# thelondonsmiths/Solex_ser_recon_EN

Hardware: AMD Instinct MI355X
Metric: SER frames/sec end-to-end (decode→clahe) + %HBM roofline, 1/2/4/8 MI355X (higher is better)
Workload: dtype u16

## Files before the change

include/shg_hip.h:

```cpp
#ifndef SHG_HIP_H
#define SHG_HIP_H

#include <stddef.h>
#include <stdint.h>

#ifdef __cplusplus
extern "C" {
#endif

#define SHG_ABI_VERSION 16

#define SHG_E_ARG        (-1)
#define SHG_E_WORKSPACE  (-2)
#define SHG_E_UNSUPPORTED (-3)
#define SHG_E_VALUE      (-4)
#define SHG_E_TYPE       (-5)
#define SHG_E_LINALG     (-6)
#define SHG_E_RUNTIME    (-7)
#define SHG_E_QHULL      (-8)
#define SHG_E_ASSERT     (-9)
#define SHG_E_INDEX      (-10)

typedef void* shg_stream_t;

// ... 239 lines not shown
int shg_flood_stats_f64(const double* image, const double* blurred, int64_t n, double very_bright,
                        double* stats, uint32_t* counts, void* workspace, shg_stream_t stream);
int shg_flood_stats_lerp_f64(const double* image, const double* blurred, int64_t n,
                             const double* order_stats, double gamma, double* stats, uint32_t* counts,
                             void* workspace, shg_stream_t stream);

size_t shg_canny_workspace_bytes(int64_t h, int64_t w);
int shg_canny_masks_f64(const double* blurred, int64_t h, int64_t w, double flood_thresh,
                        const double* host_gauss_weights, int radius, double low, double high,
                        uint8_t* low_mask, uint8_t* high_mask, void* workspace, size_t workspace_bytes,
                        shg_stream_t stream);

size_t shg_edge_components_workspace_bytes(int64_t h, int64_t w);
int shg_edge_components(const uint8_t* low_mask, const uint8_t* high_mask, int64_t h, int64_t w,
                        int32_t* out_idx, int32_t* out_root, int32_t* out_count,
                        void* workspace, size_t workspace_bytes, shg_stream_t stream);

size_t shg_contrast_stats_workspace_bytes(int tiles);
size_t shg_contrast_stats_workspace_bytes_for(int64_t h, int64_t w, int tiles);
int shg_contrast_stats_u16(const uint16_t* frame, int64_t h, int64_t w, int64_t pitch, double clip_limit,
                           int tiles, uint16_t* cl1, int64_t cl1_pitch, const int64_t* ranks_frame2,
                           const int64_t* ranks_cl13, double* out5, void* workspace, size_t workspace_bytes,
                           shg_stream_t stream);
int shg_contrast_products_u16(const uint16_t* frame, int64_t frame_pitch, const uint16_t* cl1, int64_t cl1_pitch,
                              int64_t h, int64_t w, const double* lo_hi6, uint16_t* high_contrast,
                              uint16_t* protus, uint16_t* cc, int64_t dst_pitch, int64_t disc_x0,
                              int64_t disc_y0, int64_t disc_r, shg_stream_t stream);
int shg_contrast_products_vec_fits(const uint16_t* frame, int64_t frame_pitch, const uint16_t* cl1, int64_t cl1_pitch,
                                   int64_t h, int64_t w, const uint16_t* high_contrast, const uint16_t* protus,
                                   const uint16_t* cc, int64_t dst_pitch);

int shg_limb_fused_fits(int64_t sh, int64_t sw, int k);
size_t shg_limb_prepare_workspace_bytes(int64_t sh, int64_t sw, int k);
int shg_limb_prepare(const uint16_t* img, int64_t h, int64_t w, int64_t pitch, int k, const int64_t* host_ranks4, double gamma99,
                     double* packed, const uint32_t** keys_out, void* workspace, size_t workspace_bytes, shg_stream_t stream);
size_t shg_limb_edges_workspace_bytes(int64_t sh, int64_t sw);
int shg_limb_edges(const uint32_t* keys, int64_t sh, int64_t sw, int k, double flood_thresh, const double* host_gauss_weights,
                   int radius, double low, double high, int32_t* comp, void* workspace, size_t workspace_bytes, shg_stream_t stream);


size_t shg_stage_mean_fit_workspace_bytes(int64_t n_frames, int64_t height, int64_t width, int bytes_per_px);
size_t shg_stage_mean_fit_host_bytes(int64_t height, int64_t width);
int shg_stage_mean_fit(const void* stack, int64_t n_frames, int64_t height, int64_t width, int bytes_per_px,
                       int64_t frame_stride_px, const uint64_t* sum_in, const uint16_t* max_in, int64_t n_total,
                       uint16_t* mean_out, uint16_t* max_out, int64_t* host_y12, double* host_p4, double* host_fit,
                       int32_t* host_trace_sharp, uint8_t* host_mask_good, void* workspace, size_t workspace_bytes,
// ... 167 lines not shown
```

solex_ser_recon_en_amd/_lib.py:

```python
import ctypes
import os
from ctypes import c_double, c_int, c_int32, c_int64, c_size_t, c_uint16, c_uint32, c_void_p

import torch

_HERE = os.path.dirname(os.path.abspath(__file__))
LIB_PATH = os.path.join(_HERE, 'csrc', 'libshg_hip.so')

if not os.path.exists(LIB_PATH):
    raise ImportError(
        'libshg_hip.so is missing (%s). Build it with `python -c "import __graft_entry__ as g; g.build()"` or '
        '`make -C solex_ser_recon_en_amd/csrc`. There is no CPU fallback for the SHG hot path.' % LIB_PATH)

lib = ctypes.CDLL(LIB_PATH)

P = c_void_p
PD = ctypes.POINTER(c_double)
PI64 = ctypes.POINTER(c_int64)


class ScanRequest(ctypes.Structure):
    _fields_ = [('struct_bytes', c_uint32), ('start_phase', c_int32),
                ('stack', P), ('n_frames', c_int64), ('height', c_int64), ('width', c_int64), ('frame_stride_px', c_int64),
                ('bytes_per_px', c_int32), ('flip_x', c_int32),
# ... 94 lines not shown
                                  c_int64, P, P]),
    'shg_warp_rows_wide_fits': (c_int, [P, c_int64, c_int64, c_int64, c_double, c_double, c_double, P, c_int64, c_int64, c_int64]),
    'shg_rowpair_logratio_stats': (c_int, [P, c_int64, c_int64, c_int64, c_int64, c_int64, P, P, P, P, P]),
    'shg_rowpair_logratio_stats_mirrored': (c_int, [P, c_int64, c_int64, c_int64, c_int64, c_int64, P, P, P, P, P, P]),
    'shg_line_order_stats_u16': (c_int, [P, c_int64, c_int64, c_int64, c_int, c_int64, c_int64, P, P, P]),
    'shg_scale_rows_u16': (c_int, [P, c_int64, c_int64, c_int64, P, P, P, c_int64, P]),
    'shg_scale_rows_vec_fits': (c_int, [P, c_int64, c_int64, c_int64, P, c_int64]),
    'shg_correlate1d_rows_f64': (c_int, [P, c_int64, c_int64, P, c_int, c_int, P, P]),
    'shg_lin_filter_row_sums': (c_int, [P, c_int64, c_int64, c_int64, P, P, P, P, P, c_int, P, P, P]),
    'shg_lin_filter_apply': (c_int, [P, c_int64, c_int64, c_int64, P, P, P, c_int, c_int, P, P, P, P, c_int, P, c_int64, P]),
    'shg_crop_pad_u16': (c_int, [P, c_int64, c_int64, c_int64, P, c_int64, c_int64, c_int64, c_int64, c_int64,
                                 c_int, P]),
    'shg_clahe_workspace_bytes': (c_size_t, [c_int, c_int]),
    'shg_clahe_workspace_bytes_for': (c_size_t, [c_int64, c_int64, c_int, c_int]),
    'shg_clahe': (c_int, [P, c_int64, c_int64, c_int64, c_int, c_double, c_int, P, c_int64, P, c_size_t, P]),
    'shg_hist': (c_int, [P, c_int64, c_int64, c_int64, c_int, P, P]),
    'shg_select_u16_workspace_bytes': (c_size_t, [c_int]),
    'shg_select_u16': (c_int, [P, c_int64, c_int64, c_int64, ctypes.POINTER(c_int64), c_int, P, P, c_size_t, P]),
    'shg_rescale_u16': (c_int, [P, c_int64, c_int64, c_int64, c_double, c_double, c_double, P, c_int64, P]),
    'shg_rescale_u8': (c_int, [P, c_int64, c_int64, c_int64, c_double, c_double, c_double, P, c_int64, P]),
    'shg_contrast_stats_workspace_bytes': (c_size_t, [c_int]),
    'shg_contrast_stats_workspace_bytes_for': (c_size_t, [c_int64, c_int64, c_int]),
    'shg_contrast_stats_u16': (c_int, [P, c_int64, c_int64, c_int64, c_double, c_int, P, c_int64, P, P, P, P, c_size_t, P]),
    'shg_contrast_products_u16': (c_int, [P, c_int64, P, c_int64, c_int64, c_int64, P, P, P, P, c_int64, c_int64, c_int64, c_int64, P]),
    'shg_contrast_products_vec_fits': (c_int, [P, c_int64, P, c_int64, c_int64, c_int64, P, P, P, c_int64]),
    'shg_fill_disc_u16': (c_int, [P, c_int64, c_int64, c_int64, c_int64, c_int64, c_int64, c_uint16, P, P]),
    'shg_downscale_mean_u16': (c_int, [P, c_int64, c_int64, c_int64, c_int, P, P]),
    'shg_box_blur_f64': (c_int, [P, c_int64, c_int64, c_int, P, P, P]),
    'shg_box_blur_key_f64': (c_int, [P, c_int64, c_int64, c_int, P, P, P, P]),
    'shg_select_keys_workspace_bytes': (c_size_t, [c_int]),
    'shg_select_keys_u32': (c_int, [ctypes.POINTER(c_void_p), c_int64, ctypes.POINTER(c_int64), ctypes.POINTER(c_int), c_int, P, P, c_size_t, P]),
    'shg_select_workspace_bytes': (c_size_t, [c_int]),
    'shg_select_f64': (c_int, [P, c_int64, ctypes.POINTER(c_int64), c_int, P, P, c_size_t, P]),
    'shg_select_multi_f64': (c_int, [ctypes.POINTER(c_void_p), c_int64, ctypes.POINTER(c_int64), c_int, P, P, c_size_t, P]),
    'shg_flood_stats_f64': (c_int, [P, P, c_int64, c_double, P, P, P, P]),
    'shg_flood_stats_lerp_f64': (c_int, [P, P, c_int64, P, c_double, P, P, P, P]),
    'shg_edge_components_workspace_bytes': (c_size_t, [c_int64, c_int64]),
    'shg_edge_components': (c_int, [P, P, c_int64, c_int64, P, P, P, P, c_size_t, P]),
    'shg_canny_workspace_bytes': (c_size_t, [c_int64, c_int64]),
    'shg_canny_masks_f64': (c_int, [P, c_int64, c_int64, c_double, ctypes.POINTER(c_double), c_int, c_double, c_double, P, P, P,
                                    c_size_t, P]),
    'shg_limb_fused_fits': (c_int, [c_int64, c_int64, c_int]),
    'shg_limb_prepare_workspace_bytes': (c_size_t, [c_int64, c_int64, c_int]),
    'shg_limb_prepare': (c_int, [P, c_int64, c_int64, c_int64, c_int, PI64, c_double, P, ctypes.POINTER(c_void_p), P, c_size_t, P]),
    'shg_limb_edges_workspace_bytes': (c_size_t, [c_int64, c_int64]),
    'shg_limb_edges': (c_int, [P, c_int64, c_int64, c_int, c_double, PD, c_int, c_double, c_double, P, P, c_size_t, P]),
# ... 200 lines not shown
```

solex_ser_recon_en_amd/csrc/clahe.hip:

```cpp
#include <stdlib.h>
#include <type_traits>
#include <algorithm>
#include "shg_common.h"

namespace {
template <typename T>
__device__ __forceinline__ T* zdisk(T* p, size_t zs, uint32_t z) {
    return reinterpret_cast<T*>(reinterpret_cast<char*>(const_cast<typename std::remove_const<T>::type*>(p)) + (size_t)z * zs);
}

constexpr int HIST16 = 65536;
constexpr int SEL_SLOTS = 8;
constexpr int SEL_NW = 8;
struct SelWin { uint32_t w0_cur, w0_next, max, pad; };
constexpr int SEL_WIN_SLOTS = 8;
constexpr int SEL_WIN_WORDS = SEL_WIN_SLOTS * SEL_NW * 256;
__device__ __forceinline__ uint32_t sel_window_origin(const SelWin* st) {
    const uint32_t w0 = __hip_atomic_load(&st->w0_cur, __ATOMIC_RELAXED, __HIP_MEMORY_SCOPE_AGENT);
    return w0 > 256u - SEL_NW ? 256u - SEL_NW : w0;
}
constexpr int SLICE_PX = 32768;
constexpr int kFusedMaxSliceRows = 2048;

template <typename T>
// ... 66 lines not shown
    return (uint32_t)min(q, 65535);
}
__device__ __forceinline__ double row_factor_for_fma(double c) {
    if (c != c) return 0.0;
    if (c > 0x1p+960) return 65536.0;
    if (c < -0x1p+960) return -4294967296.0;
    return c;
}

struct HistSlicesArgs {
    shg::PtrBatch imgs;
    int64_t h, w, pitch;
    int tiles;
    int64_t th, tw;
    uint32_t* part;
    size_t zs;
    int slice_rows, vec;
    FusedSrc fs;
    int clip, chunk_rows;
};

__device__ __forceinline__ int64_t mirror101(int64_t i, int64_t n) { return 2 * (n - 1) - i; }

template <bool FUSED, int BITS> __global__ __launch_bounds__(1024) void k_tile_hist16_slices(const HistSlicesArgs kargs) {
    const shg::PtrBatch& imgs = kargs.imgs;
    const int64_t h = kargs.h, w = kargs.w, pitch = kargs.pitch, th = kargs.th, tw = kargs.tw;
    const int tiles = kargs.tiles, slice_rows = kargs.slice_rows, vec = kargs.vec;
    uint32_t* __restrict__ part = kargs.part;
    const size_t zs = kargs.zs;
    const FusedSrc& fs = kargs.fs;
    extern __shared__ uint32_t lh[];
    const uint16_t* __restrict__ img = imgs.at<const uint16_t>(blockIdx.z);
    part = zdisk(part, zs, blockIdx.z);
    const int tile = blockIdx.y;
    const int64_t ty = tile / tiles, tx = tile % tiles;
    const int ya = (int)blockIdx.x * slice_rows;
    const int yb = min((int)th, ya + slice_rows) - 1;
    for (int i = threadIdx.x; i < HIST16 / 8; i += 1024) reinterpret_cast<uint4*>(lh)[i] = make_uint4(0, 0, 0, 0);
    double* cf = reinterpret_cast<double*>(lh + HIST16 / 2);
    const uint16_t* __restrict__ raw = nullptr;
    uint16_t* __restrict__ fin = nullptr;
    __shared__ uint32_t fill_s;
    const bool scaled = FUSED && fs.c != nullptr;
    if (FUSED) {
        raw = fs.raw.at<const uint16_t>(blockIdx.z);
        fin = imgs.at<uint16_t>(blockIdx.z);
        const double* c = scaled ? fs.c + (int64_t)blockIdx.z * h : nullptr;
        for (int i = threadIdx.x; i <= yb - ya; i += 1024) {
            int64_t r = ty * th + ya + i;
            if (r >= h) r = mirror101(r, h);
            cf[i] = scaled ? row_factor_for_fma(c[r]) : 1.0;
        }
        if (threadIdx.x == 0) fill_s = scaled ? scale_px(raw[0], c[0]) : (uint32_t)raw[0];
    }
    __syncthreads();
    const int chunk_rows = BITS == 16 ? slice_rows : kargs.chunk_rows;
    const uint32_t clip2 = (uint32_t)kargs.clip;
    for (int ca = ya; ca <= yb; ca += chunk_rows) {
        const int cb = min(yb, ca + chunk_rows - 1);
        if (BITS != 16 && ca != ya) {
            __syncthreads();
            for (int i = threadIdx.x; i < HIST16 / 8; i += 1024) {
                uint4 q = reinterpret_cast<uint4*>(lh)[i];
                uint32_t* d = reinterpret_cast<uint32_t*>(&q);
#pragma unroll
                for (int j = 0; j < 4; ++j) d[j] = min(d[j] & 0xffffu, clip2) | (min(d[j] >> 16, clip2) << 16);
                reinterpret_cast<uint4*>(lh)[i] = q;
            }
            __syncthreads();
        }
        const int lane = threadIdx.x & 63, wave = threadIdx.x >> 6;
        const int twi = (int)tw;
        const int64_t xbase = tx * tw;
        auto count = [&](uint32_t v) { atomicAdd(&lh[v >> 1], 1u << ((v & 1u) << 4)); };
        if (vec) {
            const int64_t xa = xbase, xb = min(xbase + tw, w);
            const int64_t xa8 = (xa + 7) & ~(int64_t)7, xb8 = max(xb & ~(int64_t)7, xa8);
            const int nvr = (int)((xb8 - xa8) / 8);
            const int n_head = (int)(min(xa8, xb) - xa), n_tail = (int)(xb - max(xb8, xa + n_head)), n_edge = n_head + n_tail + (int)(xbase + tw - xb);
            {
                const uint32_t nvr_u = (uint32_t)nvr, total_v = (uint32_t)(cb - ca + 1) * nvr_u;
                const float inv_nvr = nvr > 0 ? 1.0f / (float)nvr : 0.0f;
                constexpr int U = 4;
                for (uint32_t i0 = threadIdx.x; i0 < total_v; i0 += 1024u * U) {
                    uint4 q[U];
                    int64_t yv[U];
                    uint32_t vv[U], rowv[U];
                    bool borderv[U];
#pragma unroll
                    for (int u = 0; u < U; ++u) {
                        const uint32_t i = i0 + 1024u * u < total_v ? i0 + 1024u * u : i0;
                        uint32_t r = (uint32_t)((float)i * inv_nvr);
                        r -= (r * nvr_u > i) ? 1u : 0u;
                        r += ((r + 1u) * nvr_u <= i) ? 1u : 0u;
                        rowv[u] = r;
                        vv[u] = i - r * nvr_u;
                        int64_t y = ty * th + ca + (int64_t)r;
                        borderv[u] = y >= h;
                        if (borderv[u]) y = mirror101(y, h);
                        yv[u] = y;
                        const uint16_t* srow = FUSED ? raw + y * fs.raw_pitch : img + y * pitch;
                        q[u] = reinterpret_cast<const uint4*>(srow + xa8)[vv[u]];
                    }
#pragma unroll
                    for (int u = 0; u < U; ++u) {
                        if (i0 + 1024u * u >= total_v) break;
                        uint32_t d[4] = {q[u].x, q[u].y, q[u].z, q[u].w};
                        if (FUSED) {
                            if (scaled) {
                                const double cy = cf[ca - ya + (int)rowv[u]], kc = cy * 0x1p+52;
#pragma unroll
                                for (int j = 0; j < 4; ++j) d[j] = (scale_px_fma(d[j] & 0xffffu, cy, kc) & 0xffffu) | (scale_px_fma(d[j] >> 16, cy, kc) << 16);
                            }
                            if (!borderv[u]) reinterpret_cast<uint4*>(fin + yv[u] * pitch + xa8)[vv[u]] = make_uint4(d[0], d[1], d[2], d[3]);
                        }
#pragma unroll
                        for (int j = 0; j < 4; ++j) { count(d[j] & 0xffffu); count(d[j] >> 16); }
                    }
                }
            }
            for (int e = threadIdx.x; e < (cb - ca + 1) * n_edge; e += 1024) {
                const int rr = e / n_edge, l = e - rr * n_edge, yy = ca + rr;
                int64_t y = ty * th + yy;
                const bool border_row = y >= h;
                if (border_row) y = mirror101(y, h);
                const int64_t x = l < n_head ? xa + l : (l < n_head + n_tail ? xb - n_tail + (l - n_head) : xb + (l - n_head - n_tail));
                const bool border_col = x >= w;
                const int64_t xr = border_col ? mirror101(x, w) : x;
                uint32_t v = (FUSED ? raw + y * fs.raw_pitch : img + y * pitch)[xr];
                if (FUSED) {
                    const double cy = cf[yy - ya];
                    if (scaled) v = scale_px_fma(v, cy, cy * 0x1p+52) & 0xffffu;
                    if (!border_col && !border_row) fin[y * pitch + x] = (uint16_t)v;
                }
                count(v);
            }
        } else {
            for (int yy = ca + wave; yy <= cb; yy += 16) {
                int64_t y = ty * th + yy;
                const bool border_row = y >= h;
                if (border_row) y = mirror101(y, h);
                const uint16_t* row = FUSED ? raw + y * fs.raw_pitch : img + y * pitch;
                const double cy = FUSED ? cf[yy - ya] : 1.0, kc = cy * 0x1p+52;
// ... 1324 lines not shown
    bool ranks_done = false;
};

struct SelectRequest {
    Disks disks;
    int64_t h, w, pitch;
    const int64_t* ranks; int n_ranks;
    double* out; int out_zstride;
    void* workspace; size_t workspace_bytes; shg_stream_t stream;
    ClaheResult after = {};
};

enum class Route { Atomics8, Atomics16, Slices16, Slices8, Slices4 };
inline bool is_slices(Route r) { return r >= Route::Slices16; }

struct Plan {
    int err; char msg[120];
    Route route;
    ClaheLayout lay;
    int ntiles, clip;
    int64_t th, tw, area;
    float lut_scale;
    int bits, hist_vec;
    int64_t slice_rows, slices, chunk_rows;
    bool window;
    bool lut_all_tiles;
    int64_t lut_rank[2];
    int blend_px, blend_rounds, blend_tiled;
    bool blend_counts;
    uint32_t blend_tiles_x, blend_blocks;
};

#define PLAN_REQUIRE(cond, code, ...) \
    do { if (!(cond)) { p.err = (code); snprintf(p.msg, sizeof(p.msg), __VA_ARGS__); return p; } } while (0)

inline Plan plan_clahe(const ClaheRequest& r, const Tuning& tune) {
    Plan p = {};
    const Disks& d = r.disks;
    const int64_t h = r.im.h, w = r.im.w, pitch = r.im.pitch, dst_pitch = r.im.dst_pitch;
    const int tiles = r.im.tiles, bytes_per_px = r.im.bytes_per_px;
    PLAN_REQUIRE(h > 0 && w > 0 && pitch >= w && dst_pitch >= w, SHG_E_ARG, "shg_clahe: bad image size");
    PLAN_REQUIRE(bytes_per_px == 1 || bytes_per_px == 2, SHG_E_ARG, "shg_clahe: bytes_per_px must be 1 or 2");
    PLAN_REQUIRE(tiles >= 1 && tiles <= 16, SHG_E_UNSUPPORTED, "shg_clahe: tiles must be in 1..16");
    PLAN_REQUIRE(h < 65536, SHG_E_UNSUPPORTED, "shg_clahe: more than 65535 rows");
    p.lay = clahe_layout(h, w, tiles, bytes_per_px);
    PLAN_REQUIRE(r.workspace_bytes >= p.lay.small, SHG_E_WORKSPACE, "shg_clahe: workspace too small");
// ... 26 lines not shown
    int64_t slice_px = (d.n >= tune.big_from && tune.slice_px > SLICE_PX && tune.slice_px <= 65535) ? tune.slice_px : SLICE_PX;
    if (sat && tune.sat_px) slice_px = tune.sat_px;
    p.chunk_rows = slice_rows_of(tw, 65280);
    p.slice_rows = slice_rows_of(tw, slice_px);
    if (sat) {
        const int64_t max_slices = std::min<int64_t>(256, p.lay.n_slices * (16 / p.bits));
        if (!tune.sat_px) {
            int64_t best = 1, best_cost = INT64_MAX;
            for (int64_t sl = 1; sl <= std::min<int64_t>(max_slices, th); ++sl) {
                const int64_t rows = ceil_div(th, sl);
                if (d.fused && rows > kFusedMaxSliceRows) continue;
                const int64_t cost = ceil_div(ceil_div(th, rows) * p.ntiles * (int64_t)d.n, shg::kCUs) * (rows * tw + 8192);
                if (cost < best_cost) { best_cost = cost; best = rows; }
            }
            p.slice_rows = best;
        }
        if (ceil_div(th, p.slice_rows) > max_slices) p.slice_rows = ceil_div(th, max_slices);
        if (d.fused) p.slice_rows = std::min<int64_t>(p.slice_rows, kFusedMaxSliceRows);
    }
    p.slices = ceil_div(th, p.slice_rows);
    PLAN_REQUIRE(!d.fused || p.slice_rows <= kFusedMaxSliceRows, SHG_E_ARG, "shg_clahe: the fused histogram's slices hold at most %d rows", kFusedMaxSliceRows);
    const uintptr_t ptr_bits = d.bits_of(d.src) | d.bits_of(d.dst);
    p.hist_vec = tw >= 64 && pitch % 8 == 0 && (ptr_bits & 15) == 0 && (!d.fused || d.from_in_vectors(w));
    p.window = r.sel_hist && r.want_window;
    p.lut_all_tiles = p.ntiles <= 16 && d.n >= 8;

    const bool vec = (ptr_bits & 7) == 0 && pitch % 4 == 0 && dst_pitch % 4 == 0;
    p.blend_px = vec ? 4 : 1;
    p.blend_counts = vec && r.sel_hist;
    p.blend_rounds = p.blend_counts ? 4 : 1;
    p.blend_tiles_x = 1u;
    if (p.blend_counts && tune.interp_tiled) {
        const int shape = tune.interp_shape;
        const int lw = shape ? (shape & 15) : 2, wx = shape ? ((shape >> 4) & 15) : 2;
        const bool px8 = (shape ? ((shape >> 8) & 1) != 0 : d.n >= 4) && (ptr_bits & 15) == 0 && pitch % 8 == 0 && dst_pitch % 8 == 0;
        p.blend_px = px8 ? 8 : 4;
        const int64_t wg_px = (int64_t)p.blend_px << (lw + wx), wg_rows = (int64_t)(64 >> lw) * (4 >> wx);
        p.blend_tiles_x = (uint32_t)ceil_div(w, wg_px);
        p.blend_tiled = 0x10000 | lw | (wx << 8);
        p.blend_blocks = p.blend_tiles_x * (uint32_t)ceil_div(h, wg_rows * p.blend_rounds);
    } else {
        p.blend_blocks = (unsigned)ceil_div(ceil_div(w, p.blend_px) * h, 256 * (int64_t)p.blend_rounds);
    }
    return p;
}
#undef PLAN_REQUIRE

template <typename Args> using Kernel = void (*)(Args);
inline Kernel<HistSlicesArgs> pick_hist_slices(bool fused, int bits) {
    if (fused) return bits == 16 ? k_tile_hist16_slices<true, 16> : bits == 8 ? k_tile_hist16_slices<true, 8> : k_tile_hist16_slices<true, 4>;
    return bits == 16 ? k_tile_hist16_slices<false, 16> : bits == 8 ? k_tile_hist16_slices<false, 8> : k_tile_hist16_slices<false, 4>;
}
inline Kernel<HistReduceArgs> pick_hist_reduce(int bits) { return bits == 16 ? k_hist_reduce : bits == 8 ? k_hist_reduce_sat<8> : k_hist_reduce_sat<4>; }
inline Kernel<LutBlocksArgs> pick_lut_blocks(bool sat, bool all_tiles) {
    if (all_tiles) return sat ? k_tile_lut16_blocks<true, true> : k_tile_lut16_blocks<false, true>;
    return sat ? k_tile_lut16_blocks<true, false> : k_tile_lut16_blocks<false, false>;
}
inline Kernel<InterpVmArgs> pick_interp_vm(int px, bool counts, bool t2) {
    if (counts && px == 8) return t2 ? k_clahe_interp_vm<8, true, true> : k_clahe_interp_vm<8, true, false>;
    if (counts) return t2 ? k_clahe_interp_vm<4, true, true> : k_clahe_interp_vm<4, true, false>;
    if (px == 4) return t2 ? k_clahe_interp_vm<4, false, true> : k_clahe_interp_vm<4, false, false>;
    return t2 ? k_clahe_interp_vm<1, false, true> : k_clahe_interp_vm<1, false, false>;
}

void ensure_lds_attr() {
    static const bool done = [] {
        auto allow = [](auto kernel, size_t lds) {
            (void)hipFuncSetAttribute(reinterpret_cast<const void*>(kernel), hipFuncAttributeMaxDynamicSharedMemorySize, (int)lds);
        };
        for (int bits : {16, 8, 4}) {
            allow(pick_hist_slices(false, bits), HIST16 * 2);
            allow(pick_hist_slices(true, bits), HIST16 * 2 + kFusedMaxSliceRows * 8);
        }
        allow(pick_lut_blocks(true, true), 2048 * 16 * 2);
        allow(pick_lut_blocks(false, true), 2048 * 16 * 2);
        allow(k_tile_hist16, HIST16 * 2);
        allow(k_image_hist16, HIST16 * 2);
        allow(k_tile_lut16_lds, (HIST16 + HIST16 / 64) * 2);
        return true;
    }();
    (void)done;
}

ClaheResult clahe_slices(const ClaheRequest& r, const Plan& p) {
    ClaheResult out;
    ensure_lds_attr();
    hipStream_t st = shg::as_stream(r.stream);
    const Disks& d = r.disks;
    const Shape& im = r.im;
    char* ws = static_cast<char*>(r.workspace);
    uint32_t* hist = reinterpret_cast<uint32_t*>(ws);
    uint16_t* lut = reinterpret_cast<uint16_t*>(ws + p.lay.lut);
    uint32_t* part = reinterpret_cast<uint32_t*>(ws + p.lay.slices);
    uint32_t* chunk_tile = reinterpret_cast<uint32_t*>(ws + p.lay.chunk);
    int32_t* se = reinterpret_cast<int32_t*>(ws + p.lay.se);
    const unsigned nz = (unsigned)d.n, ntiles = (unsigned)p.ntiles;
    const bool sat = p.bits != 16;
    { SHG_PROF("clahe_hist", st);
      const HistSlicesArgs ha{d.src, im.h, im.w, im.pitch, im.tiles, p.th, p.tw, part, d.zs, (int)p.slice_rows, p.hist_vec, d.fused ? d.from : FusedSrc{}, p.clip, (int)p.chunk_rows};
      const size_t lds = HIST16 * 2 + (d.fused ? (size_t)p.slice_rows * 8 : 0);
      if ((out.err = shg::launch(pick_hist_slices(d.fused, p.bits), dim3((unsigned)p.slices, ntiles, nz), dim3(1024), lds, st, ha, "k_tile_hist16_slices")))
          return out;
      const HistReduceArgs ra{part, (int)p.slices, p.clip, hist, chunk_tile, se, d.zs, r.sel_hist, r.sel_hist ? SEL_SLOTS * r.sel_stride : 0, p.window ? 1 : 0};
      if ((out.err = shg::launch(pick_hist_reduce(p.bits), dim3(p.bits == 8 ? 64u : 32u, ntiles, nz), dim3(sat ? 256u : 1024u), 0, st, ra, sat ? "k_hist_reduce_sat" : "k_hist_reduce")))
          return out;
      out.sel_zeroed = r.sel_hist != nullptr; }
    { SHG_PROF("clahe_lut", st);
      LutBlocksArgs la{hist, se, p.clip, p.lut_scale, lut, d.zs, 0, {0, 0}, nullptr, 0, nullptr, 0, (int)p.area, p.ntiles, BorderPx{{}, im.h, im.w, im.pitch, im.h, im.w}};
      if (r.ranks) {
          la.border = BorderPx{d.src, im.h, im.w, im.pitch, p.th * im.tiles, p.tw * im.tiles};
          la.n_ranks = 2, la.rank[0] = p.lut_rank[0], la.rank[1] = p.lut_rank[1];
          la.chunk_sums = chunk_tile, la.chunk_sets = p.ntiles;
          la.ranks_out = r.ranks->out, la.ranks_zstride = r.ranks->out_zstride;
          out.ranks_done = true;
      }
      const dim3 grid(32u + (unsigned)la.n_ranks, p.lut_all_tiles ? 1u : ntiles, nz);
      const size_t lds = p.lut_all_tiles ? (size_t)2048 * p.ntiles * sizeof(uint16_t) : 0;
      if ((out.err = shg::launch(pick_lut_blocks(sat, p.lut_all_tiles), grid, dim3(1024), lds, st, la, "k_tile_lut16_blocks"))) return out; }
    { SHG_PROF("clahe_interp", st);
      const InterpVmArgs ia{d.src, im.h, im.w, im.pitch, im.tiles, 1.0f / (float)p.tw, 1.0f / (float)p.th, lut, d.dst, im.dst_pitch, p.blend_rounds,
                            p.blend_counts ? r.sel_hist : nullptr, p.blend_counts ? r.sel_stride : 0, d.zs, p.blend_tiled, p.blend_tiles_x, p.blend_counts && p.window ? 1 : 0};
      if ((out.err = shg::launch(pick_interp_vm(p.blend_px, p.blend_counts, im.tiles == 2), dim3(p.blend_blocks, 1u, nz), dim3(256), 0, st, ia, "k_clahe_interp_vm")))
          return out;
      out.pass0_done = p.blend_counts;
// ... 224 lines not shown
        const RanksJob job{{ranks.v[0], ranks.v[1]}, out5 + 5 * i0, 5};
        ClaheRequest cr{d, Shape{h, w, pitch, cl1_pitch, 2, clip_limit, tiles}, ws, lay.select2, stream};
        cr.want_chunks = true;
        cr.sel_hist = reinterpret_cast<uint32_t*>(ws + lay.select3);
        cr.sel_stride = (1 + 3) * 256;
        cr.want_window = tune.window_for(m);
        cr.ranks = &job;
        const ClaheResult c = clahe_impl(cr, tune);
        if (c.err) return c.err;
        SHG_REQUIRE(c.chunk_tile && c.sel_zeroed, SHG_E_RUNTIME, "shg_contrast_stats_u16: the batched path did not take the slice histograms");
        if (!c.ranks_done) {
            SHG_PROF("hist_ranks", st);
            if (int e = shg::launch(k_hist_ranks, dim3(2u, 1u, (unsigned)m), dim3(1024), 0, st,
                                   HistRanksArgs{reinterpret_cast<const uint32_t*>(ws), c.chunk_tile, tiles * tiles, tiles * tiles, ranks, out5 + 5 * i0, per, 5}, "k_hist_ranks"))
                return e;
        }
        d.src = d.dst;
        SelectRequest sr{d, h, w, cl1_pitch, ranks_cl13, 3, out5 + 5 * i0 + 2, 5, cr.sel_hist, select_bytes(3), stream};
        sr.after = c;
        if (int e = select_u16_impl(sr, tune)) return e;
    }
    return 0;
}
```

solex_ser_recon_en_amd/csrc/transversalium.hip:

```cpp
#include <math.h>
#include <algorithm>
#include "shg_common.h"
#include "fast_log.h"

namespace {

constexpr int MAXN = SHG_TRANSV_MAX_COLS;
constexpr int NT = 256;

using shg::f64_key;
using shg::key_f64;

constexpr int NB = 512;
constexpr int CAP = 128;

struct alignas(16) Scratch {
    uint32_t hist[2][256];
    int64_t wave_tot[2][4];
    int64_t pick[2][3];
    unsigned long long found[2];
    unsigned long long cand[CAP];
    unsigned long long kmin, kmax;
    uint32_t n_cand;
    double red[8];
// ... 159 lines not shown
#pragma unroll
            for (int r = 0; r < 2; ++r) {
                const uint32_t rk = (uint32_t)(r ? rank_hi : rank_lo);
                if (run <= rk && rk < p[7]) {
                    uint32_t b = 0, before = run, in = c[0];
#pragma unroll
                    for (int k = 0; k < 7; ++k) {
                        const bool past = rk >= p[k];
                        b += past ? 1u : 0u;
                        before = past ? p[k] : before;
                        in = past ? c[k + 1] : in;
                    }
                    sc.pick32[4 * r] = 8u * (uint32_t)lane + b;
                    sc.pick32[4 * r + 1] = before;
                    sc.pick32[4 * r + 2] = in;
                }
            }
        }
        __syncthreads();
        const int b0 = (int)sc.pick32[0], b1 = (int)sc.pick32[4];
        const uint32_t base = sc.pick32[1];
        const uint32_t cnt = sc.pick32[2] + (b1 != b0 ? sc.pick32[6] : 0u);
        if (cnt <= (uint32_t)CAP) {
            const double from = b0 == 0 ? -__builtin_huge_val() : (double)b0, to = b1 == NB - 1 ? __builtin_huge_val() : (double)(b1 + 1);
            sweep(n, [&](int i) {
                const double v = val(i);
                const double t = place(v);
                if (in_play(v) && t >= from && t < to) cand[atomicAdd(&sc.n_cand, 1u)] = v;
            });
            __syncthreads();
            const int m = (int)sc.n_cand;
            if (tid < m) {
                const double mine = cand[tid];
                uint32_t r = base;
                for (int j = 0; j < m; ++j) {
                    const double o = cand[j];
                    r += (o < mine || (o == mine && j < tid)) ? 1u : 0u;
                }
                if (r == (uint32_t)rank_lo) sc.vfound[0] = mine;
                if (r == (uint32_t)rank_hi) sc.vfound[1] = mine;
            }
            __syncthreads();
            out_lo = sc.vfound[0];
            out_hi = sc.vfound[1];
            __syncthreads();
            return true;
        }
        if (b0 != b1) return false;
        if (tid == 0) { sc.kmin = ~0ull; sc.kmax = 0ull; }
        __syncthreads();
        uint64_t mn = ~0ull, mx = 0ull;
// ... 154 lines not shown
        }
        if (odd) sc.nonfinite = 1;
    } else {
        bool odd = false;
        for (int i = threadIdx.x; i < n; i += NT) {
            const double q = ((double)r1[i] * f1) / ((double)r0[i] * f0);
            const double x = (q >= 2.2250738585072014e-308 && q <= 1.7976931348623157e308) ? shg::log_normal(q) : log(q);
            if (x != x) sc.bad = 1;
            odd = odd || !(fabs(x) <= 1.7976931348623157e308);
            vals[i] = x;
            sum1 += x;
            sum2 = fma(x, x, sum2);
        }
        if (odd) sc.nonfinite = 1;
    }
    float rough1 = (float)sum1, rough2 = (float)sum2;
    block_sum2_rough(rough1, rough2, sc.redf);
    __syncthreads();
    if (sc.bad) {
        emit(__builtin_nan(""));
        return;
    }
    const bool finite = !sc.nonfinite;
    const float per_n = __builtin_amdgcn_rcpf((float)n);
    const float meanf = rough1 * per_n, varf = rough2 * per_n - meanf * meanf;
    const double mean = (double)meanf;
    const double sigma = varf > 0.0f ? (double)__builtin_amdgcn_sqrtf(varf) : 0.0;
    const int lo = (n & 1) ? (n >> 1) : (n >> 1) - 1, hi = n >> 1;
    double va, vb;
    auto general = [&](auto key) {
        uint64_t ka, kb;
        select2(key, n, lo, hi, sc, ka, kb);
        va = key_f64(ka);
        vb = key_f64(kb);
    };
    const double kMedSpan = 1.0, kMadSpan = 1.0;
    auto row_val = [&](int i) { return vals[i]; };
    if (!(finite && select2_buckets(row_val, n, lo, hi, mean - kMedSpan * sigma, mean + kMedSpan * sigma, sc, va, vb)))
        general([&](int i) { return f64_key(vals[i]); });
    const double med = (n & 1) ? va : (va + vb) / 2.0;
    if (!finite) {
        for (int i = threadIdx.x; i < n; i += NT) {
            const double dv = fabs(vals[i] - med);
            if (dv != dv) sc.bad = 1;
        }
        __syncthreads();
        if (sc.bad) {
            emit(__builtin_nan(""));
            return;
        }
    }
    auto dev_val = [&](int i) { return fabs(vals[i] - med); };
    if (!(finite && select2_buckets(dev_val, n, lo, hi, 0.0, kMadSpan * sigma, sc, va, vb)))
        general([&](int i) { return f64_key(fabs(vals[i] - med)); });
    const double mdev = (n & 1) ? va : (va + vb) / 2.0;
    const double twice = 2.0 * mdev;
    const bool all = !(mdev != 0.0);
    double s = 0.0;
    uint32_t kept = 0;
    sweep<false>(n, [&](int i) {
        const double x = vals[i];
        const bool keep = all || fabs(x - med) < twice;
        kept += (uint32_t)__popcll(__ballot(keep));
        if (keep) s += x;
    });
    s = wave_sum(s);
    __syncthreads();
    if ((threadIdx.x & 63) == 0) { sc.red[threadIdx.x >> 6] = s; sc.kept[threadIdx.x >> 6] = kept; }
    __syncthreads();
    s = (sc.red[0] + sc.red[1]) + (sc.red[2] + sc.red[3]);
    const double cnt = (double)((sc.kept[0] + sc.kept[1]) + (sc.kept[2] + sc.kept[3]));
    emit(s / cnt);
}

__global__ __launch_bounds__(256) void k_scale_rows(shg::PtrBatch imgs, int64_t w, int64_t pitch,
                                                    const double* __restrict__ c, const double* __restrict__ row_factor,
// ... 25 lines not shown
    uint16_t* __restrict__ dst = dsts.at<uint16_t>(blockIdx.z);
    c += (int64_t)blockIdx.z * h;
    const bool factored = row_factor != nullptr;
    const bool full = x + 8 <= w;
    uint4 q[SCALE_ROWS];
    double cy[SCALE_ROWS], fy[SCALE_ROWS];
#pragma unroll
    for (int rr = 0; rr < SCALE_ROWS; ++rr) {
        const int64_t y = ya + rr < h ? ya + rr : h - 1;
        if (full) q[rr] = *reinterpret_cast<const uint4*>(img + y * pitch + x);
        cy[rr] = c[y];
        fy[rr] = factored ? row_factor[y] : 1.0;
    }
#pragma unroll
    for (int rr = 0; rr < SCALE_ROWS; ++rr) {
        const int64_t y = ya + rr;
        if (y >= h) break;
        const double cyr = cy[rr], fyr = fy[rr];
        auto one = [&](uint32_t px) {
            double v = (double)px;
            if (factored) v = v * fyr;
            v = v * cyr;
            v = v > 65535.0 ? 65535.0 : v;
            return (uint32_t)(int)v;
        };
        if (full) {
            uint4 o;
            o.x = one(q[rr].x & 0xffffu) | (one(q[rr].x >> 16) << 16);
            o.y = one(q[rr].y & 0xffffu) | (one(q[rr].y >> 16) << 16);
            o.z = one(q[rr].z & 0xffffu) | (one(q[rr].z >> 16) << 16);
            o.w = one(q[rr].w & 0xffffu) | (one(q[rr].w >> 16) << 16);
            *reinterpret_cast<uint4*>(dst + y * dst_pitch + x) = o;
        } else {
            for (int64_t i = x; i < w; ++i) dst[y * dst_pitch + i] = (uint16_t)one(img[y * pitch + i]);
        }
    }
}

constexpr int CORR_MAXR = 1024;

struct CorrelateArgs {
    const double* src;
    int64_t n;
    const double* weights;
    int radius, symmetric;
    double* dst;
};
// ... 201 lines not shown
```

solex_ser_recon_en_amd/ops.py:

```python
import ctypes

import numpy as np
import torch

from . import _lib
from ._lib import lib


def _stream():
    return torch._C._cuda_getCurrentRawStream(torch.cuda.current_device())


def _dev(t, what):
    if not isinstance(t, torch.Tensor) or not t.is_cuda:
        raise RuntimeError('%s must be a GPU tensor: the SHG hot path has no CPU fallback' % what)
    return t


def _img(t, what, dtype=None):
    _dev(t, what)
    if t.dim() != 2 or (t.shape[1] > 1 and t.stride(1) != 1):
        raise ValueError('%s must be a 2-D image with contiguous rows' % what)
    if dtype is not None and t.dtype != dtype:
        raise TypeError('%s must be %s, got %s' % (what, dtype, t.dtype))
# ... 358 lines not shown
    if need == 0:
        raise ValueError('clahe: unsupported tile count %r' % (tiles,))
    ws = torch.empty(need, dtype=torch.uint8, device=img.device)
    out = pitched_u16(h, w, img.device) if bpp == 2 else torch.empty((h, w), dtype=torch.uint8, device=img.device)
    _lib.check(lib.shg_clahe(ptr, h, w, pitch, bpp, float(clip_limit), int(tiles), out.data_ptr(), out.stride(0),
                             ws.data_ptr(), need, _stream()), 'shg_clahe')
    return out


def contrast_stats_u16(frame, ranks_frame, ranks_cl1, out5, clip_limit=0.8, tiles=2, small_workspace=False):
    import ctypes
    ptr, h, w, pitch = _img(frame, 'frame', torch.uint16)
    need = (lib.shg_contrast_stats_workspace_bytes(int(tiles)) if small_workspace
            else lib.shg_contrast_stats_workspace_bytes_for(h, w, int(tiles)))
    if need == 0:
        raise ValueError('contrast_stats: unsupported tile count %r' % (tiles,))
    ws = torch.empty(need, dtype=torch.uint8, device=frame.device)
    cl1 = pitched_u16(h, w, frame.device)
    rf = (ctypes.c_int64 * 2)(*[int(r) for r in ranks_frame])
    rc = (ctypes.c_int64 * 3)(*[int(r) for r in ranks_cl1])
    _lib.check(lib.shg_contrast_stats_u16(ptr, h, w, pitch, float(clip_limit), int(tiles), cl1.data_ptr(), cl1.stride(0), rf, rc,
                                          out5.data_ptr(), ws.data_ptr(), need, _stream()), 'shg_contrast_stats_u16')
    return cl1


def contrast_products_u16(frame, cl1, lo_hi6, disc=None):
    import ctypes
    ptr, h, w, pitch = _img(frame, 'frame', torch.uint16)
    cptr, ch, cw, cpitch = _img(cl1, 'cl1', torch.uint16)
    if (ch, cw) != (h, w):
        raise ValueError('frame and cl1 must share one shape')
    store = torch.empty((3, h, (w + 63) // 64 * 64), dtype=torch.uint16, device=frame.device)
    hc, protus, cc = store[0, :, :w], store[1, :, :w], store[2, :, :w]
    bounds = (ctypes.c_double * 6)(*[float(v) for v in lo_hi6])
    x0, y0, r = (int(v) for v in disc) if disc is not None else (0, 0, 0)
    _lib.check(lib.shg_contrast_products_u16(ptr, pitch, cptr, cpitch, h, w, bounds, hc.data_ptr(), protus.data_ptr(), cc.data_ptr(),
                                             store.stride(1), x0, y0, r, _stream()), 'shg_contrast_products_u16')
    return hc, protus, cc


def histogram(img):
    _dev(img, 'img')
    bpp = 2 if img.dtype == torch.uint16 else 1
    if img.dtype not in (torch.uint16, torch.uint8):
        raise TypeError('histogram needs uint8 or uint16')
    ptr, h, w, pitch = _img(img, 'img')
# ... 635 lines not shown
```

Baseline: 6.076 million.

## Add early-load fused histogram variant, batched contrast stats API, and NaN-robust median steering

Adds an EARLY variant of the fused CLAHE tile-histogram kernel for small batches (n<=3). It issues the first vector pixel loads before writing row factors to shared memory and hitting the barrier, so that global-load latency overlaps the factor setup. The change also exposes a batched multi-frame contrast-stats entry point with crop and scaling, which lets callers process several frames in one call. Separately, it makes the robust median/MAD selection use bucket steering with finite-only statistics when non-finite values are present, and adjusts bucket boundary and pixel masking semantics. Together these add kernel variants and more surface area to keep correct.

```diff
diff --git a/include/shg_hip.h b/include/shg_hip.h
--- a/include/shg_hip.h
+++ b/include/shg_hip.h
@@ -285,6 +285,11 @@
                            int tiles, uint16_t* cl1, int64_t cl1_pitch, const int64_t* ranks_frame2,
                            const int64_t* ranks_cl13, double* out5, void* workspace, size_t workspace_bytes,
                            shg_stream_t stream);
+int shg_contrast_stats_frames_u16(const uint16_t* const* host_raw, int64_t k, int64_t h, int64_t w, int64_t raw_pitch,
+                                  const double* factors, int64_t out_w, int64_t sx0, int64_t dx0, int64_t ncopy,
+                                  double clip_limit, int tiles, uint16_t* const* host_final, uint16_t* const* host_cl1,
+                                  int64_t out_pitch, const int64_t* ranks_frame2, const int64_t* ranks_cl13, double* out5,
+                                  void* workspace, size_t workspace_bytes, shg_stream_t stream);
 int shg_contrast_products_u16(const uint16_t* frame, int64_t frame_pitch, const uint16_t* cl1, int64_t cl1_pitch,
                               int64_t h, int64_t w, const double* lo_hi6, uint16_t* high_contrast,
                               uint16_t* protus, uint16_t* cc, int64_t dst_pitch, int64_t disc_x0,
diff --git a/solex_ser_recon_en_amd/_lib.py b/solex_ser_recon_en_amd/_lib.py
--- a/solex_ser_recon_en_amd/_lib.py
+++ b/solex_ser_recon_en_amd/_lib.py
@@ -140,6 +140,8 @@
     'shg_contrast_stats_workspace_bytes': (c_size_t, [c_int]),
     'shg_contrast_stats_workspace_bytes_for': (c_size_t, [c_int64, c_int64, c_int]),
     'shg_contrast_stats_u16': (c_int, [P, c_int64, c_int64, c_int64, c_double, c_int, P, c_int64, P, P, P, P, c_size_t, P]),
+    'shg_contrast_stats_frames_u16': (c_int, [P, c_int64, c_int64, c_int64, c_int64, P, c_int64, c_int64, c_int64, c_int64, c_double, c_int,
+                                              P, P, c_int64, P, P, P, P, c_size_t, P]),
     'shg_contrast_products_u16': (c_int, [P, c_int64, P, c_int64, c_int64, c_int64, P, P, P, P, c_int64, c_int64, c_int64, c_int64, P]),
     'shg_contrast_products_vec_fits': (c_int, [P, c_int64, P, c_int64, c_int64, c_int64, P, P, P, c_int64]),
     'shg_fill_disc_u16': (c_int, [P, c_int64, c_int64, c_int64, c_int64, c_int64, c_int64, c_uint16, P, P]),
diff --git a/solex_ser_recon_en_amd/csrc/clahe.hip b/solex_ser_recon_en_amd/csrc/clahe.hip
--- a/solex_ser_recon_en_amd/csrc/clahe.hip
+++ b/solex_ser_recon_en_amd/csrc/clahe.hip
@@ -112,7 +112,8 @@
 
 __device__ __forceinline__ int64_t mirror101(int64_t i, int64_t n) { return 2 * (n - 1) - i; }
 
-template <bool FUSED, int BITS> __global__ __launch_bounds__(1024) void k_tile_hist16_slices(const HistSlicesArgs kargs) {
+template <bool FUSED, int BITS, bool EARLY = false> __global__ __launch_bounds__(1024) void k_tile_hist16_slices(const HistSlicesArgs kargs) {
+    static_assert(FUSED || !EARLY, "EARLY is a variant of the fused kernel");
     const shg::PtrBatch& imgs = kargs.imgs;
     const int64_t h = kargs.h, w = kargs.w, pitch = kargs.pitch, th = kargs.th, tw = kargs.tw;
     const int tiles = kargs.tiles, slice_rows = kargs.slice_rows, vec = kargs.vec;
@@ -132,18 +133,45 @@
     uint16_t* __restrict__ fin = nullptr;
     __shared__ uint32_t fill_s;
     const bool scaled = FUSED && fs.c != nullptr;
+    const bool early = EARLY && vec != 0;
+    double early_c[2] = {1.0, 1.0};
+    static_assert(kFusedMaxSliceRows <= 2 * 1024, "a thread carries two of a slice's row factors");
     if (FUSED) {
         raw = fs.raw.at<const uint16_t>(blockIdx.z);
         fin = imgs.at<uint16_t>(blockIdx.z);
         const double* c = scaled ? fs.c + (int64_t)blockIdx.z * h : nullptr;
-        for (int i = threadIdx.x; i <= yb - ya; i += 1024) {
-            int64_t r = ty * th + ya + i;
-            if (r >= h) r = mirror101(r, h);
-            cf[i] = scaled ? row_factor_for_fma(c[r]) : 1.0;
-        }
-        if (threadIdx.x == 0) fill_s = scaled ? scale_px(raw[0], c[0]) : (uint32_t)raw[0];
-    }
-    __syncthreads();
+        if (early) {
+#pragma unroll
+            for (int k = 0; k < 2; ++k) {
+                const int i = (int)threadIdx.x + 1024 * k;
+                if (scaled && i <= yb - ya) {
+                    int64_t r = ty * th + ya + i;
+                    if (r >= h) r = mirror101(r, h);
+                    early_c[k] = c[r];
+                }
+            }
+        } else {
+            for (int i = threadIdx.x; i <= yb - ya; i += 1024) {
+                int64_t r = ty * th + ya + i;
+                if (r >= h) r = mirror101(r, h);
+                cf[i] = scaled ? row_factor_for_fma(c[r]) : 1.0;
+            }
+            if (threadIdx.x == 0) fill_s = scaled ? scale_px(raw[0], c[0]) : (uint32_t)raw[0];
+        }
+    }
+    bool pending = early;
+    auto park_factors = [&]() {
+#pragma unroll
+        for (int k = 0; k < 2; ++k) {
+            const int i = (int)threadIdx.x + 1024 * k;
+            double c = early_c[k];
+            asm volatile("" : "+v"(c));
+            if (i <= yb - ya) cf[i] = scaled ? row_factor_for_fma(c) : 1.0;
+        }
+        __syncthreads();
+        pending = false;
+    };
+    if (!early) __syncthreads();
     const int chunk_rows = BITS == 16 ? slice_rows : kargs.chunk_rows;
     const uint32_t clip2 = (uint32_t)kargs.clip;
     for (int ca = ya; ca <= yb; ca += chunk_rows) {
@@ -172,14 +200,14 @@
                 const uint32_t nvr_u = (uint32_t)nvr, total_v = (uint32_t)(cb - ca + 1) * nvr_u;
                 const float inv_nvr = nvr > 0 ? 1.0f / (float)nvr : 0.0f;
                 constexpr int U = 4;
-                for (uint32_t i0 = threadIdx.x; i0 < total_v; i0 += 1024u * U) {
+                for (uint32_t i0 = threadIdx.x; (EARLY ? i0 - threadIdx.x : i0) < total_v; i0 += 1024u * U) {
                     uint4 q[U];
                     int64_t yv[U];
                     uint32_t vv[U], rowv[U];
                     bool borderv[U];
 #pragma unroll
                     for (int u = 0; u < U; ++u) {
-                        const uint32_t i = i0 + 1024u * u < total_v ? i0 + 1024u * u : i0;
+                        const uint32_t i = i0 + 1024u * u < total_v ? i0 + 1024u * u : (EARLY && i0 >= total_v ? 0u : i0);
                         uint32_t r = (uint32_t)((float)i * inv_nvr);
                         r -= (r * nvr_u > i) ? 1u : 0u;
                         r += ((r + 1u) * nvr_u <= i) ? 1u : 0u;
@@ -192,6 +220,12 @@
                         const uint16_t* srow = FUSED ? raw + y * fs.raw_pitch : img + y * pitch;
                         q[u] = reinterpret_cast<const uint4*>(srow + xa8)[vv[u]];
                     }
+                    if (EARLY && pending) park_factors();
+                    if (EARLY) {
+                        asm volatile("" :: "v"(q[0].x), "v"(q[0].y), "v"(q[0].z), "v"(q[0].w), "v"(q[1].x), "v"(q[1].y), "v"(q[1].z), "v"(q[1].w));
+                        asm volatile("" :: "v"(q[2].x), "v"(q[2].y), "v"(q[2].z), "v"(q[2].w), "v"(q[3].x), "v"(q[3].y), "v"(q[3].z), "v"(q[3].w));
+                        static_assert(U == 4, "the vectors named above");
+                    }
 #pragma unroll
                     for (int u = 0; u < U; ++u) {
                         if (i0 + 1024u * u >= total_v) break;
@@ -209,6 +243,7 @@
                     }
                 }
             }
+            if (EARLY && pending) park_factors();
             for (int e = threadIdx.x; e < (cb - ca + 1) * n_edge; e += 1024) {
                 const int rr = e / n_edge, l = e - rr * n_edge, yy = ca + rr;
                 int64_t y = ty * th + yy;
@@ -1579,6 +1614,7 @@
     int64_t th, tw, area;
     float lut_scale;
     int bits, hist_vec;
+    bool hist_early;
     int64_t slice_rows, slices, chunk_rows;
     bool window;
     bool lut_all_tiles;
@@ -1651,6 +1687,7 @@
     PLAN_REQUIRE(!d.fused || p.slice_rows <= kFusedMaxSliceRows, SHG_E_ARG, "shg_clahe: the fused histogram's slices hold at most %d rows", kFusedMaxSliceRows);
     const uintptr_t ptr_bits = d.bits_of(d.src) | d.bits_of(d.dst);
     p.hist_vec = tw >= 64 && pitch % 8 == 0 && (ptr_bits & 15) == 0 && (!d.fused || d.from_in_vectors(w));
+    p.hist_early = d.fused && p.hist_vec && d.n <= 3;
     p.window = r.sel_hist && r.want_window;
     p.lut_all_tiles = p.ntiles <= 16 && d.n >= 8;
 
@@ -1676,7 +1713,8 @@
 #undef PLAN_REQUIRE
 
 template <typename Args> using Kernel = void (*)(Args);
-inline Kernel<HistSlicesArgs> pick_hist_slices(bool fused, int bits) {
+inline Kernel<HistSlicesArgs> pick_hist_slices(bool fused, int bits, bool early = false) {
+    if (fused && early) return bits == 16 ? k_tile_hist16_slices<true, 16, true> : bits == 8 ? k_tile_hist16_slices<true, 8, true> : k_tile_hist16_slices<true, 4, true>;
     if (fused) return bits == 16 ? k_tile_hist16_slices<true, 16> : bits == 8 ? k_tile_hist16_slices<true, 8> : k_tile_hist16_slices<true, 4>;
     return bits == 16 ? k_tile_hist16_slices<false, 16> : bits == 8 ? k_tile_hist16_slices<false, 8> : k_tile_hist16_slices<false, 4>;
 }
@@ -1700,6 +1738,7 @@
         for (int bits : {16, 8, 4}) {
             allow(pick_hist_slices(false, bits), HIST16 * 2);
             allow(pick_hist_slices(true, bits), HIST16 * 2 + kFusedMaxSliceRows * 8);
+            allow(pick_hist_slices(true, bits, true), HIST16 * 2 + kFusedMaxSliceRows * 8);
         }
         allow(pick_lut_blocks(true, true), 2048 * 16 * 2);
         allow(pick_lut_blocks(false, true), 2048 * 16 * 2);
@@ -1728,7 +1767,7 @@
     { SHG_PROF("clahe_hist", st);
       const HistSlicesArgs ha{d.src, im.h, im.w, im.pitch, im.tiles, p.th, p.tw, part, d.zs, (int)p.slice_rows, p.hist_vec, d.fused ? d.from : FusedSrc{}, p.clip, (int)p.chunk_rows};
       const size_t lds = HIST16 * 2 + (d.fused ? (size_t)p.slice_rows * 8 : 0);
-      if ((out.err = shg::launch(pick_hist_slices(d.fused, p.bits), dim3((unsigned)p.slices, ntiles, nz), dim3(1024), lds, st, ha, "k_tile_hist16_slices")))
+      if ((out.err = shg::launch(pick_hist_slices(d.fused, p.bits, p.hist_early), dim3((unsigned)p.slices, ntiles, nz), dim3(1024), lds, st, ha, "k_tile_hist16_slices")))
           return out;
       const HistReduceArgs ra{part, (int)p.slices, p.clip, hist, chunk_tile, se, d.zs, r.sel_hist, r.sel_hist ? SEL_SLOTS * r.sel_stride : 0, p.window ? 1 : 0};
       if ((out.err = shg::launch(pick_hist_reduce(p.bits), dim3(p.bits == 8 ? 64u : 32u, ntiles, nz), dim3(sat ? 256u : 1024u), 0, st, ra, sat ? "k_hist_reduce_sat" : "k_hist_reduce")))
@@ -1999,3 +2038,21 @@
     }
     return 0;
 }
+
+extern "C" int shg_contrast_stats_frames_u16(const uint16_t* const* host_raw, int64_t k, int64_t h, int64_t w, int64_t raw_pitch,
+                                             const double* factors, int64_t out_w, int64_t sx0, int64_t dx0, int64_t ncopy,
+                                             double clip_limit, int tiles, uint16_t* const* host_final, uint16_t* const* host_cl1,
+                                             int64_t out_pitch, const int64_t* ranks_frame2, const int64_t* ranks_cl13, double* out5,
+                                             void* workspace, size_t workspace_bytes, shg_stream_t stream) {
+    SHG_REQUIRE(host_raw && host_final && host_cl1 && ranks_frame2 && ranks_cl13 && out5 && workspace && k > 0, SHG_E_ARG,
+                "shg_contrast_stats_frames_u16: null pointer");
+    SHG_REQUIRE(h > 0 && w > 0 && out_w > 0 && raw_pitch >= w && out_pitch >= out_w, SHG_E_ARG, "shg_contrast_stats_frames_u16: bad image size");
+    SHG_REQUIRE(sx0 >= 0 && dx0 >= 0 && ncopy >= 0 && sx0 + ncopy <= w && dx0 + ncopy <= out_w, SHG_E_ARG,
+                "shg_contrast_stats_frames_u16: the copied columns leave the frame or the image");
+    for (int64_t i = 0; i < k; ++i) SHG_REQUIRE(host_raw[i], SHG_E_ARG, "shg_contrast_stats_frames_u16: null frame");
+    SHG_REQUIRE(shg::contrast_stats_batches(h, out_w, tiles, clip_limit) && workspace_bytes >= (size_t)k * shg_contrast_stats_workspace_bytes_for(h, out_w, tiles),
+                SHG_E_UNSUPPORTED, "shg_contrast_stats_frames_u16: shape or workspace outside the batched route");
+    const shg::FrameSource from = {host_raw, raw_pitch, factors, sx0, dx0, ncopy};
+    return shg::contrast_stats_batch(host_final, k, h, out_w, out_pitch, clip_limit, tiles, host_cl1, out_pitch, ranks_frame2, ranks_cl13, out5, workspace,
+                                     workspace_bytes, stream, &from);
+}
diff --git a/solex_ser_recon_en_amd/csrc/transversalium.hip b/solex_ser_recon_en_amd/csrc/transversalium.hip
--- a/solex_ser_recon_en_amd/csrc/transversalium.hip
+++ b/solex_ser_recon_en_amd/csrc/transversalium.hip
@@ -205,11 +205,11 @@
         const uint32_t base = sc.pick32[1];
         const uint32_t cnt = sc.pick32[2] + (b1 != b0 ? sc.pick32[6] : 0u);
         if (cnt <= (uint32_t)CAP) {
-            const double from = b0 == 0 ? -__builtin_huge_val() : (double)b0, to = b1 == NB - 1 ? __builtin_huge_val() : (double)(b1 + 1);
+            const double from = b0 == 0 ? -__builtin_huge_val() : (double)b0, to = b1 == NB - 1 ? __builtin_nan("") : (double)(b1 + 1);
             sweep(n, [&](int i) {
                 const double v = val(i);
                 const double t = place(v);
-                if (in_play(v) && t >= from && t < to) cand[atomicAdd(&sc.n_cand, 1u)] = v;
+                if (in_play(v) && t >= from && !(t >= to)) cand[atomicAdd(&sc.n_cand, 1u)] = v;
             });
             __syncthreads();
             const int m = (int)sc.n_cand;
@@ -410,7 +410,27 @@
         return;
     }
     const bool finite = !sc.nonfinite;
-    const float per_n = __builtin_amdgcn_rcpf((float)n);
+    bool steered = finite;
+    float n_steer = (float)n;
+    if (!finite) {
+        float s1 = 0.0f, s2 = 0.0f, cnt = 0.0f, none = 0.0f;
+        for (int i = threadIdx.x; i < n; i += NT) {
+            const double x = vals[i];
+            if (fabs(x) <= 1.7976931348623157e308) {
+                const float xf = (float)x;
+                s1 += xf;
+                s2 = fmaf(xf, xf, s2);
+                cnt += 1.0f;
+            }
+        }
+        block_sum2_rough(s1, s2, sc.redf);
+        block_sum2_rough(cnt, none, sc.redf);
+        rough1 = s1;
+        rough2 = s2;
+        n_steer = cnt;
+        steered = cnt > 0.0f;
+    }
+    const float per_n = __builtin_amdgcn_rcpf(n_steer);
     const float meanf = rough1 * per_n, varf = rough2 * per_n - meanf * meanf;
     const double mean = (double)meanf;
     const double sigma = varf > 0.0f ? (double)__builtin_amdgcn_sqrtf(varf) : 0.0;
@@ -424,7 +444,7 @@
     };
     const double kMedSpan = 1.0, kMadSpan = 1.0;
     auto row_val = [&](int i) { return vals[i]; };
-    if (!(finite && select2_buckets(row_val, n, lo, hi, mean - kMedSpan * sigma, mean + kMedSpan * sigma, sc, va, vb)))
+    if (!(steered && select2_buckets(row_val, n, lo, hi, mean - kMedSpan * sigma, mean + kMedSpan * sigma, sc, va, vb)))
         general([&](int i) { return f64_key(vals[i]); });
     const double med = (n & 1) ? va : (va + vb) / 2.0;
     if (!finite) {
@@ -439,7 +459,7 @@
         }
     }
     auto dev_val = [&](int i) { return fabs(vals[i] - med); };
-    if (!(finite && select2_buckets(dev_val, n, lo, hi, 0.0, kMadSpan * sigma, sc, va, vb)))
+    if (!(steered && select2_buckets(dev_val, n, lo, hi, 0.0, kMadSpan * sigma, sc, va, vb)))
         general([&](int i) { return f64_key(fabs(vals[i] - med)); });
     const double mdev = (n & 1) ? va : (va + vb) / 2.0;
     const double twice = 2.0 * mdev;
@@ -511,7 +531,7 @@
             if (factored) v = v * fyr;
             v = v * cyr;
             v = v > 65535.0 ? 65535.0 : v;
-            return (uint32_t)(int)v;
+            return (uint32_t)(int)v & 0xffffu;
         };
         if (full) {
             uint4 o;
diff --git a/solex_ser_recon_en_amd/ops.py b/solex_ser_recon_en_amd/ops.py
--- a/solex_ser_recon_en_amd/ops.py
+++ b/solex_ser_recon_en_amd/ops.py
@@ -404,6 +404,37 @@
     _lib.check(lib.shg_contrast_stats_u16(ptr, h, w, pitch, float(clip_limit), int(tiles), cl1.data_ptr(), cl1.stride(0), rf, rc,
                                           out5.data_ptr(), ws.data_ptr(), need, _stream()), 'shg_contrast_stats_u16')
     return cl1
+
+
+def contrast_stats_frames_u16(raws, factors, ranks_frame, ranks_cl1, crop=None, clip_limit=0.8, tiles=2):
+    import ctypes
+    k = len(raws)
+    ptr, h, w, pitch = _img(raws[0], 'raw', torch.uint16)
+    for f in raws[1:]:
+        if _img(f, 'raw', torch.uint16)[1:] != (h, w, pitch):
+            raise ValueError('contrast_stats_frames: the frames must share one shape and row pitch')
+    dev = raws[0].device
+    out_w, sx0, dx0, ncopy = (int(v) for v in crop) if crop is not None else (w, 0, 0, w)
+    fac = None
+    if factors is not None:
+        fac = factors if isinstance(factors, torch.Tensor) else torch.as_tensor(np.ascontiguousarray(factors, dtype=np.float64))
+        fac = fac.to(dev).contiguous()
+        if fac.shape != (k, h) or fac.dtype != torch.float64:
+            raise ValueError('factors must be float64 [k, h]')
+    need = k * lib.shg_contrast_stats_workspace_bytes_for(h, out_w, int(tiles))
+    if need == 0:
+        raise ValueError('contrast_stats_frames: unsupported tile count %r' % (tiles,))
+    ws = torch.empty(need, dtype=torch.uint8, device=dev)
+    finals = [pitched_u16(h, out_w, dev) for _ in range(k)]
+    cl1s = [pitched_u16(h, out_w, dev) for _ in range(k)]
+    out5 = torch.empty((k, 5), dtype=torch.float64, device=dev)
+    arr = lambda ts: (ctypes.c_void_p * k)(*[t.data_ptr() for t in ts])
+    rf = (ctypes.c_int64 * 2)(*[int(r) for r in ranks_frame])
+    rc = (ctypes.c_int64 * 3)(*[int(r) for r in ranks_cl1])
+    _lib.check(lib.shg_contrast_stats_frames_u16(arr(raws), k, h, w, pitch, None if fac is None else fac.data_ptr(), out_w, sx0, dx0, ncopy,
+                                                 float(clip_limit), int(tiles), arr(finals), arr(cl1s), finals[0].stride(0), rf, rc,
+                                                 out5.data_ptr(), ws.data_ptr(), need, _stream()), 'shg_contrast_stats_frames_u16')
+    return finals, cl1s, out5
 
 
 def contrast_products_u16(frame, cl1, lo_hi6, disc=None):
```

After: 6.087 million, median of 2. About the same (+0.2%).
